# google/zopfli

Measured on AMD Instinct MI355X. Metric: input MB/s at numiterations=15 (gzip, bit-exact vs reference), higher is better.
Workload: dtype u8 (f32/f64 cost DP); 1 GPU; class-T synthetic (text-like, the enwik8 stand-in) 100000000 B per GPU, numiterations=15, blocksplitting=0, gzip, BASELINE configs[1]; total_bytes=100000000, master_blocks=100, gather=none (one rank)

## Files before the change

### zopfli_amd/csrc/device/zmx_hip.hip

```cpp
#include <hip/hip_runtime.h>

#include <algorithm>
#include <atomic>
#include <cmath>
#include <cstdio>
#include <cstdlib>
#include <cstring>
#include <mutex>
#include <string>
#include <unordered_map>
#include <vector>

#include "zmx_kernels.h"
#include "zmx_match2.h"
#ifdef ZMX_EXPERIMENTS
#include "zmx_match3.h"
#include "zmx_match4.h"
#else
#define BK_CH 32768u
#endif
#include "zmx_match5.h"
#include "zmx_dp4.h"
#include "zmx_dp5.h"
#include "zmx_encode.h"
// ... 540 lines not shown
#ifdef ZMX_EXPERIMENTS
  HIPCHK(hipFuncSetAttribute(reinterpret_cast<const void*>(k_bucket), hipFuncAttributeMaxDynamicSharedMemorySize,
                             BK_LDS_BYTES));
#endif
  *out = c;
  return 0;
}

int zmx_ctx_set_priority(zmx_ctx* c, int level) {
  DeviceGuard dev_guard(c->device);
  HIPCHK(dev_guard.err);
  const int k = level > 0 ? 1 : level < 0 ? 2 : 0;
  if (!c->alt_stream[0][0]) { c->alt_stream[0][0] = c->stream; c->alt_stream[0][1] = c->stream2; }
  if (k && !c->alt_stream[k][1]) {
    int least = 0, greatest = 0;
    HIPCHK(hipDeviceGetStreamPriorityRange(&least, &greatest));
    for (int i = 0; i < 2; ++i) {
      if (c->alt_stream[k][i]) continue;
      HIPCHK(hipStreamCreateWithPriority(&c->alt_stream[k][i], hipStreamDefault, k == 1 ? greatest : least));
    }
  }
  HIPCHK(hipStreamSynchronize(c->stream));
  HIPCHK(hipStreamSynchronize(c->stream2));
  c->stream = c->alt_stream[k][0];
  c->stream2 = c->alt_stream[k][1];
  return 0;
}

void zmx_ctx_destroy(zmx_ctx* c) {
  if (!c) return;
  DeviceGuard dev_guard(c->device);
  if (c->h_stage) (void)hipHostFree(c->h_stage);
  for (auto& f : c->pinned_free) (void)hipHostFree(f.first);
  for (auto& f : c->pool_free) (void)hipFree(f.first);
  DevCached(c).fetch_sub(c->pool_free_bytes, std::memory_order_relaxed);
  for (auto& f : c->pool_live) (void)hipFree(c->guard_live.count(f.first) ? static_cast<unsigned char*>(f.first) - kGuardBytes : f.first);
  (void)hipFree(c->d_guard_tab);
  for (int i = 0; i < 4; ++i) if (c->ev[i]) (void)hipEventDestroy(c->ev[i]);
  for (int i = 0; i < 2; ++i) if (c->ev2[i]) (void)hipEventDestroy(c->ev2[i]);
  if (c->alt_stream[0][0]) {
    for (int k = 0; k < 3; ++k) for (int i = 0; i < 2; ++i) if (c->alt_stream[k][i]) (void)hipStreamDestroy(c->alt_stream[k][i]);
  } else {
    if (c->stream2) (void)hipStreamDestroy(c->stream2);
    if (c->stream) (void)hipStreamDestroy(c->stream);
  }
  delete c;
}

int zmx_set_input(zmx_ctx* c, const unsigned char* in, size_t insize) {
  DeviceGuard dev_guard(c->device);
  HIPCHK(dev_guard.err);
  if (insize + kInputPad > c->in_cap) {
    PoolFree(c, c->d_in);
    c->d_in = nullptr;
    c->in_cap = insize + kInputPad;
    HIPCHK(PoolAllocT(c, &c->d_in, c->in_cap, "d_in"));
  }
  if (insize) HIPCHK(hipMemcpyAsync(c->d_in, in, insize, hipMemcpyHostToDevice, c->stream));
  HIPCHK(hipMemsetAsync(c->d_in + insize, 0, kInputPad, c->stream));
  HIPCHK(hipStreamSynchronize(c->stream));
  c->insize = insize;
  c->h_in = in;
  return 0;
}

static void ReleaseTableArrays(zmx_ctx* c, zmx_tables* t, bool keep_stores) {
  auto rel = [&](auto*& p) { PoolFree(c, p); p = nullptr; };
  rel(t->d_blocks);
  rel(t->d_tile_off);
  rel(t->d_same16);
  rel(t->d_links);
  rel(t->d_sorted_alloc);
  rel(t->d_ssame);
  rel(t->d_chunk_base);
  rel(t->d_recs);
  rel(t->d_pool);
  rel(t->d_la);
  rel(t->d_dph);
  rel(t->d_block_edges);
  rel(t->d_badpos);
  rel(t->d_code_base);
  rel(t->d_codes);
  rel(t->d_wtab);
  rel(t->d_badcodes);
  rel(t->d_seg_off);
  rel(t->d_extab);
  rel(t->d_seginfo);
  rel(t->d_counters);
  rel(t->d_prof);
  rel(t->d_tasks);
  rel(t->d_task_off);
  rel(t->d_wg_tasks);
  rel(t->d_task_kind);
  rel(t->d_run_list);
  rel(t->d_wmeta);
  rel(t->d_runin);
  rel(t->d_runout);
  rel(t->d_winroff);
  rel(t->d_winflag);
  rel(t->d_win_off);
  rel(t->d_lvl);
  rel(t->d_entry);
  rel(t->d_exit);
  rel(t->d_mid);
  rel(t->d_chk);
  rel(t->d_over);
  rel(t->d_redo);
  for (int h = 0; h < 2; ++h) { rel(t->d_rank[h]); rel(t->d_bucket[h]); }
  t->d_sorted[0] = t->d_sorted[1] = nullptr;
  PinnedGive(c, &t->h_runin, t->h_runin_cap);
  PinnedGive(c, &t->h_runout, t->h_runout_cap);
  if (!keep_stores) { rel(t->d_store[0]); rel(t->d_store[1]); }
}

void zmx_tables_free(zmx_ctx* c, zmx_tables* t) {
  if (!t) return;
  DeviceGuard dev_guard(c ? c->device : 0);
  if (c && c->stream2) (void)hipStreamSynchronize(c->stream2);
  ReleaseTableArrays(c, t, false);
  delete t;
}

int zmx_tables_trim(zmx_ctx* c, zmx_tables* t) {
  if (!t) return 0;
  DeviceGuard dev_guard(c->device);
  HIPCHK(dev_guard.err);
  HIPCHK(hipStreamSynchronize(c->stream));
  HIPCHK(hipStreamSynchronize(c->stream2));
  ReleaseTableArrays(c, t, true);
  t->trimmed = true;
  return 0;
}

static unsigned EnvU32(const char* name, unsigned dflt, unsigned lo, unsigned hi) {
  const char* e = std::getenv(name);
  if (!e) return dflt;
  const long v = std::atol(e);
  return v < static_cast<long>(lo) ? lo : v > static_cast<long>(hi) ? hi : static_cast<unsigned>(v);
}
static unsigned SegL(u64 total_positions) {
  static const bool set = std::getenv("ZOPFLI_AMD_SEG_L") != nullptr;
  static const unsigned v = EnvU32("ZOPFLI_AMD_SEG_L", 4096, 0, 1u << 24) & ~63u;
  if (set) return v;
  return total_positions <= (128u << 10) ? 256u : total_positions <= (16u << 20) ? 512u : total_positions <= (48u << 20) ? 1024u : 2048u;
}
static unsigned SegHead(size_t nb) {
  static const unsigned v = EnvU32("ZOPFLI_AMD_SEG_HEAD", 0, 0, 1u << 24) & ~63u;
  return v ? v : (nb >= 48 ? 8192u : 0u);
}
static unsigned SegWarm() { static const unsigned v = (EnvU32("ZOPFLI_AMD_SEG_WARM", 512, 64, 1u << 20) + 63u) & ~63u; return v; }

static int BuildTables(zmx_ctx* c, const zmx_block* blocks, size_t nb, zmx_tables* t, zmx_tables* parent = nullptr, bool with_dp = true) {
  const int mk = MatchKernel();
  t->matches_only = !with_dp;
  t->nb = nb;
  t->blocks.resize(nb);
  t->bsize.resize(nb);
  t->store_begin[0].assign(nb, 0);
  t->store_begin[1].assign(nb, 0);
  std::vector<u32> tile_off(nb + 1, 0);
  u64 pos_off = 0, reg_off = 0, la_off = 0, max_l = 0;
  for (size_t b = 0; b < nb; ++b) {
    if (blocks[b].inend < blocks[b].instart || blocks[b].inend > c->insize) {
      return FailMsg("zmx_tables_build: block outside the resident input");
    }
    BlockDesc& d = t->blocks[b];
    d.instart = blocks[b].instart;
    d.inend = blocks[b].inend;
    d.ws = d.instart > ZMX_WINDOW ? d.instart - ZMX_WINDOW : 0;
    d.pos_off = pos_off;
    d.reg_off = reg_off;
    d.la_off = la_off;
    const u64 B = d.inend - d.instart, L = d.inend - d.ws;
    if (B > 0x7fff0000ull) return FailMsg("zmx_tables_build: block too large (positions are 32-bit)");
    t->bsize[b] = static_cast<u32>(B);
    pos_off += B;
    reg_off += (L + 7) & ~7ull;
    la_off += (B + 1 + 7) & ~7ull;
    max_l = std::max(max_l, L);
    tile_off[b + 1] = tile_off[b] + static_cast<u32>((B + MT - 1) / MT);
  }
  t->total_b = pos_off;
  t->total_l = reg_off;
  t->tile_off = tile_off;
  if (nb == 0) return 0;

  std::vector<u64> src_pos;
  std::vector<u64> link_lo;
  std::vector<u32> tile_list;
  bool reuse = parent != nullptr && parent->nb > 0 && c->h_in != nullptr && parent->d_recs != nullptr &&
               parent->total_b + pos_off < (3ull << 30);
  if (reuse) {
    src_pos.resize(nb);
    link_lo.resize(nb);
    size_t pb = 0;
    for (size_t b = 0; b < nb && reuse; ++b) {
      const BlockDesc& d = t->blocks[b];
      while (pb < parent->nb && parent->blocks[pb].inend < d.inend) ++pb;
      if (pb == parent->nb || d.instart < parent->blocks[pb].instart || d.inend > parent->blocks[pb].inend) {
        reuse = false;
        break;
      }
      const BlockDesc& pd = parent->blocks[pb];
      src_pos[b] = pd.pos_off + (d.instart - pd.instart);
      const u64 B = d.inend - d.instart;
      link_lo[b] = d.inend - d.ws;
      if (B == 0 || d.inend == pd.inend) continue;
      u64 t0 = B > ZMX_MAX_MATCH ? d.inend - ZMX_MAX_MATCH : d.instart;
      const unsigned char lastb = c->h_in[d.inend - 1];
      u64 r = d.inend - 1;
      while (r > d.instart && d.inend - r < 65600 && c->h_in[r - 1] == lastb) --r;
      if (r < t0) t0 = r;
      const u32 tile_first = static_cast<u32>((t0 - d.instart) / MT);
      for (u32 tile = tile_first; tile < tile_off[b + 1] - tile_off[b]; ++tile) {
        tile_list.push_back(tile_off[b] + tile);
      }
      const u64 first_index = d.instart + static_cast<u64>(tile_first) * MT - d.ws;
      link_lo[b] = first_index > ZMX_WINDOW ? first_index - ZMX_WINDOW : 0;
    }
  }

  HIPCHK(PoolAlloc(c, &t->d_blocks, nb));
  HIPCHK(PoolAlloc(c, &t->d_tile_off, nb + 1));
  HIPCHK(PoolAlloc(c, &t->d_same16, reg_off));
#ifdef ZMX_EXPERIMENTS
  t->buckets = mk == 3 || mk == 4;
#else
  t->buckets = false;
#endif
  t->chunk_base.assign(nb + 1, 0);
  for (size_t b = 0; b < nb; ++b) {
    const u64 L = t->blocks[b].inend - t->blocks[b].ws;
    t->chunk_base[b + 1] = t->chunk_base[b] + static_cast<u32>((L + BK_CH - 1) / BK_CH);
  }
#ifdef ZMX_EXPERIMENTS
  if (t->buckets) {
    HIPCHK(PoolAlloc(c, &t->d_sorted_alloc, 2 * reg_off + 2 * M4_PAD));
    t->d_sorted[0] = t->d_sorted_alloc + M4_PAD;
    t->d_sorted[1] = t->d_sorted[0] + reg_off + M4_PAD;
    for (int h = 0; h < 2; ++h) {
      HIPCHK(PoolAlloc(c, &t->d_rank[h], reg_off));
      HIPCHK(PoolAlloc(c, &t->d_bucket[h], static_cast<size_t>(t->chunk_base[nb]) * 32768u));
    }
    HIPCHK(PoolAlloc(c, &t->d_ssame, reg_off));
    HIPCHK(PoolAlloc(c, &t->d_chunk_base, nb + 1));
    HIPCHK(hipMemcpyAsync(t->d_chunk_base, t->chunk_base.data(), (nb + 1) * sizeof(u32), hipMemcpyHostToDevice, c->stream));
  } else
#endif
  {
    HIPCHK(PoolAlloc(c, &t->d_links, reg_off));
  }
  HIPCHK(PoolAlloc(c, &t->d_recs, pos_off * 8));
  HIPCHK(PoolAlloc(c, &t->d_la, la_off));
  HIPCHK(PoolAlloc(c, &t->d_store[0], pos_off));
  HIPCHK(PoolAlloc(c, &t->d_store[1], pos_off));
  {
    const size_t in_cost = 0, in_min = in_cost + nb * ZMX_HIST * sizeof(double), in_info = in_min + nb * sizeof(double),
                 in_slot = in_info + 3 * nb * sizeof(float);
    t->runin_bytes = in_slot + nb * sizeof(int);
    const size_t out_hist = 0, out_nsym = out_hist + nb * ZMX_HIST * sizeof(u32), out_stats = out_nsym + nb * sizeof(u32),
                 out_flags = out_stats + 8 * sizeof(u32);
    t->runout_bytes = out_flags + 4 * sizeof(u32);
    HIPCHK(PoolAlloc(c, &t->d_runin, t->runin_bytes));
    HIPCHK(PoolAlloc(c, &t->d_runout, t->runout_bytes));
    HIPCHK(PinnedTake(c, &t->h_runin, t->runin_bytes, &t->h_runin_cap));
    HIPCHK(PinnedTake(c, &t->h_runout, t->runout_bytes, &t->h_runout_cap));
    t->d_cost = reinterpret_cast<double*>(t->d_runin + in_cost);
    t->d_mincost = reinterpret_cast<double*>(t->d_runin + in_min);
    t->d_runinfo = reinterpret_cast<float*>(t->d_runin + in_info);
    t->d_slot = reinterpret_cast<int*>(t->d_runin + in_slot);
    t->d_hist = reinterpret_cast<u32*>(t->d_runout + out_hist);
    t->d_nsym = reinterpret_cast<u32*>(t->d_runout + out_nsym);
    t->d_segstats = reinterpret_cast<u32*>(t->d_runout + out_stats);
    t->d_flags = reinterpret_cast<u32*>(t->d_runout + out_flags);
    HIPCHK(hipMemsetAsync(t->d_segstats, 0, 12 * sizeof(u32), c->stream));
  }
  HIPCHK(PoolAlloc(c, &t->d_dph, pos_off));
  HIPCHK(PoolAlloc(c, &t->d_block_edges, nb));
  t->badpos_words = pos_off / 32 + 4;
  HIPCHK(PoolAlloc(c, &t->d_badpos, t->badpos_words));
  HIPCHK(PoolAlloc(c, &t->d_code_base, nb));
  HIPCHK(PoolAlloc(c, &t->d_wtab, nb * ZMX_WTAB));
  HIPCHK(PoolAlloc(c, &t->d_badcodes, nb * 40));
  HIPCHK(PoolAlloc(c, &t->d_counters, 48));
  HIPCHK(hipMemcpyAsync(t->d_blocks, t->blocks.data(), nb * sizeof(BlockDesc), hipMemcpyHostToDevice, c->stream));
  HIPCHK(hipMemcpyAsync(t->d_tile_off, tile_off.data(), (nb + 1) * sizeof(u32), hipMemcpyHostToDevice, c->stream));
  HIPCHK(hipMemsetAsync(t->d_flags, 0, 4 * sizeof(u32), c->stream));

  HIPCHK(hipEventRecord(c->ev[0], c->stream));
  PoolScope hash_tmp(c);
  u16* d_lev = nullptr;
  u16* d_tot2 = nullptr;
  u16* d_rank2 = nullptr;
  uint4* d_xrec = nullptr;
  u32* d_tot12 = nullptr;
  unsigned long long* d_energy = nullptr;
  u32* d_cmax = nullptr;
  bool skip_any = false, skip_all = false;
  double skip_positions = 0;
  unsigned long long* d_m5stats = nullptr;
  bool join_stream2 = false;
  auto launch_hash = [&](const u64* d_link_lo) -> int {
    if (max_l == 0) return 0;
    const dim3 g1(static_cast<unsigned>((max_l + 256 * SAME_CH - 1) / (256 * SAME_CH)), static_cast<unsigned>(nb));
    hipLaunchKernelGGL(k_same, g1, dim3(256), 0, c->stream, c->d_in, t->d_blocks, t->d_same16, d_link_lo);
    KCHK(c, "k_same");
    HIPCHK(hipGetLastError());
    const dim3 g2(static_cast<unsigned>((max_l + CH_EMIT - 1) / CH_EMIT), static_cast<unsigned>(nb), 2);
#ifdef ZMX_EXPERIMENTS
    if (t->buckets) {
      BucketParams kp;
      kp.in = c->d_in;
      kp.blocks = t->d_blocks;
      kp.same16 = t->d_same16;
      kp.chunk_base = t->d_chunk_base;
      kp.link_lo = d_link_lo;
      for (int h = 0; h < 2; ++h) { kp.sorted[h] = t->d_sorted[h]; kp.rank[h] = t->d_rank[h]; kp.bucket[h] = t->d_bucket[h]; }
      kp.ssame = t->d_ssame;
      hipLaunchKernelGGL(k_bucket, g2, dim3(BK_THREADS), BK_LDS_BYTES, c->stream, kp);
      KCHK(c, "k_bucket");
    } else
#endif
    {
      hipLaunchKernelGGL(k_chain, g2, dim3(64), CH_LDS_BYTES, c->stream, c->d_in, t->d_blocks, t->d_same16, t->d_links, d_link_lo);
      KCHK(c, "k_chain");
      if ((mk == 5 || mk == 0) && d_link_lo == nullptr) {
        skip_any = mk == 5;
        if (mk == 5) for (size_t b = 0; b < nb; ++b) skip_positions += static_cast<double>(t->blocks[b].inend - t->blocks[b].instart);
        const unsigned hits_chunks = static_cast<unsigned>((max_l + RK_CH - 1) / RK_CH);
        {
          static const bool rank_all = [] { const char* e = std::getenv("ZOPFLI_AMD_RANK_ALL"); return e && std::atoi(e) != 0; }();
          if (!d_energy) HIPCHK(hash_tmp.AllocT(&d_energy, nb, "d_energy"));
          if (!d_cmax && !rank_all) HIPCHK(hash_tmp.AllocT(&d_cmax, nb * static_cast<size_t>(hits_chunks) + 1, "d_cmax"));
          HIPCHK(hipMemsetAsync(d_energy, 0, nb * sizeof(unsigned long long), c->stream));
          if (d_cmax) HIPCHK(hipMemsetAsync(d_cmax, 0, (nb * static_cast<size_t>(hits_chunks) + 1) * sizeof(u32), c->stream));
          HitsParams hp;
          hp.in = c->d_in;
          hp.blocks = t->d_blocks;
          hp.same16 = t->d_same16;
          hp.energy = d_energy;
          hp.cmax = d_cmax;
          const dim3 g5(hits_chunks, static_cast<unsigned>(nb));
          hipLaunchKernelGGL(k_hits, g5, dim3(RK_THREADS), 0, c->stream, hp);
          KCHK(c, "k_hits");
        }
        if (mk == 0) {
          std::vector<unsigned long long> energy(nb);
          HIPCHK(hipMemcpyAsync(energy.data(), d_energy, nb * sizeof(unsigned long long), hipMemcpyDeviceToHost, c->stream));
          HIPCHK(hipStreamSynchronize(c->stream));
          size_t on = 0;
          for (size_t b = 0; b < nb; ++b) {
            if (energy[b] > MatchAutoHits() * (t->blocks[b].inend - t->blocks[b].ws)) {
              ++on;
              skip_positions += static_cast<double>(t->blocks[b].inend - t->blocks[b].instart);
            }
          }
          skip_any = on != 0;
          skip_all = on == nb;
        }
        if (skip_any) {
          if (!d_lev) HIPCHK(hash_tmp.AllocT(&d_lev, static_cast<size_t>(LV_N) * reg_off, "d_lev"));
          if (!d_tot2) HIPCHK(hash_tmp.AllocT(&d_tot2, 2 * reg_off, "d_tot"));
          if (!d_rank2) HIPCHK(hash_tmp.AllocT(&d_rank2, 2 * reg_off, "d_rank"));
          if (!d_tot12) HIPCHK(hash_tmp.AllocT(&d_tot12, reg_off, "d_tot12"));
          if (!d_xrec) HIPCHK(hash_tmp.AllocT(&d_xrec, 2 * reg_off, "d_xrec"));
          LevelParams lp;
          lp.in = c->d_in;
          lp.blocks = t->d_blocks;
          lp.lev = d_lev;
          lp.total_l = reg_off;
          lp.energy = mk == 0 ? d_energy : nullptr;
          lp.thr = MatchAutoHits();
          const dim3 g4(static_cast<unsigned>((max_l + LV_CH - 1) / LV_CH), static_cast<unsigned>(nb), LV_N);
          hipLaunchKernelGGL(k_levels, g4, dim3(64), 0, c->stream, lp);
          KCHK(c, "k_levels");
          RankParams rp;
          rp.in = c->d_in;
          rp.blocks = t->d_blocks;
          rp.links = t->d_links;
          rp.same16 = t->d_same16;
          rp.lev = d_lev;
          rp.total_l = reg_off;
          rp.tot = d_tot2;
          rp.rank = d_rank2;
          rp.xrec = d_xrec;
          rp.tot12 = d_tot12;
          rp.energy = lp.energy;
          rp.thr = lp.thr;
          rp.cmax = d_cmax;
          rp.cmax_stride = hits_chunks;
          const dim3 g3(static_cast<unsigned>((max_l + RK_CH - 1) / RK_CH), static_cast<unsigned>(nb));
          hipLaunchKernelGGL(k_rank2, g3, dim3(RK_THREADS), 0, c->stream, rp);
          KCHK(c, "k_rank2");
        }
      }
    }
    return 0;
  };
  {
    u64* d_link_lo = nullptr;
    if (reuse) {
      HIPCHK(hash_tmp.AllocT(&d_link_lo, nb, "d_link_lo"));
      HIPCHK(hipMemcpyAsync(d_link_lo, link_lo.data(), nb * sizeof(u64), hipMemcpyHostToDevice, c->stream));
    }
    if (launch_hash(d_link_lo) != 0) return -1;
    t->links_partial = reuse;
  }

  if (mk != 3 && !c->d_scratch) HIPCHK(PoolAllocT(c, &c->d_scratch, static_cast<size_t>(kMatchGrid) * M2_THREADS * SCRATCH_CPS, "d_scratch"));
  HIPCHK(hipEventRecord(c->ev[1], c->stream));
  double match_positions = 0;
  double m5_lane_iters = 0, m5_iters = 0;
  auto launch_match = [&](u32* pool, u32 pool_cap, u32 total_tiles, const u32* d_tiles, bool prof) -> int {
    if (total_tiles == 0) return 0;
#ifdef ZMX_EXPERIMENTS
    if (t->buckets) {
      Match3Params mp;
      mp.in = c->d_in;
      mp.blocks = t->d_blocks;
      mp.tile_off = t->d_tile_off;
      mp.nb = static_cast<u32>(nb);
      mp.total_tiles = total_tiles;
      mp.same16 = t->d_same16;
      mp.chunk_base = t->d_chunk_base;
      for (int h = 0; h < 2; ++h) { mp.sorted[h] = t->d_sorted[h]; mp.rank[h] = t->d_rank[h]; mp.bucket[h] = t->d_bucket[h]; }
      mp.ssame = t->d_ssame;
      mp.recs = t->d_recs;
      mp.pool = pool;
      mp.pool_cap = pool_cap;
      mp.counters = t->d_counters;
      mp.tile_list = d_tiles;
      mp.scratch = c->d_scratch;
      if (mk == 3) {
        if (prof) hipLaunchKernelGGL((k_match3<true>), dim3(kMatchGrid3), dim3(M3_THREADS), 0, c->stream, mp);
        else hipLaunchKernelGGL((k_match3<false>), dim3(kMatchGrid3), dim3(M3_THREADS), 0, c->stream, mp);
        KCHK(c, "k_match3");
      } else {
        if (prof) hipLaunchKernelGGL((k_match4<true>), dim3(kMatchGrid3), dim3(M4_THREADS), 0, c->stream, mp);
        else hipLaunchKernelGGL((k_match4<false>), dim3(kMatchGrid3), dim3(M4_THREADS), 0, c->stream, mp);
        KCHK(c, "k_match4");
      }
      return 0;
    }
#endif
    MatchParams mp;
    mp.in = c->d_in;
    mp.blocks = t->d_blocks;
    mp.tile_off = t->d_tile_off;
    mp.nb = static_cast<u32>(nb);
    mp.total_tiles = total_tiles;
    mp.links = t->d_links;
    mp.recs = t->d_recs;
    mp.pool = pool;
    mp.pool_cap = pool_cap;
    mp.counters = t->d_counters;
    mp.scratch = c->d_scratch;
    mp.tile_list = d_tiles;
    mp.skip_energy = nullptr;
    mp.skip_thr = 0;
    if ((mk == 5 || mk == 0) && d_tiles == nullptr && skip_any) {
      if (!c->d_scratch5) HIPCHK(PoolAllocT(c, &c->d_scratch5, static_cast<size_t>(kMatchGrid5) * M5_THREADS * SCRATCH_CPS, "d_scratch5"));
      Match5Params q;
      q.m = mp;
      q.m.scratch = c->d_scratch5;
      q.xrec = d_xrec;
      q.tot12 = d_tot12;
      q.energy = mk == 0 ? d_energy : nullptr;
      q.thr = MatchAutoHits();
      const size_t m5_waves = static_cast<size_t>(kMatchGrid5) * (M5_THREADS / 64);
      if (!d_m5stats) HIPCHK(hash_tmp.AllocT(&d_m5stats, 2 * m5_waves, "d_m5stats"));
      HIPCHK(hipMemsetAsync(d_m5stats, 0, 2 * m5_waves * sizeof(unsigned long long), c->stream));
      q.wave_stats = d_m5stats;
      {
        static const int forced = [] { const char* e = std::getenv("ZOPFLI_AMD_M5_UNIT"); return e ? std::atoi(e) : -1; }();
        const u64 waves = static_cast<u64>(kMatchGrid5) * (M5_THREADS / 64);
        q.sub_shift = forced >= 0 ? static_cast<u32>(forced > 2 ? 2 : forced) : (mp.total_tiles >= 4 * waves ? 1u : 2u);
      }
      if (mk == 5 || skip_all) {
        hipLaunchKernelGGL(k_match5, dim3(kMatchGrid5), dim3(M5_THREADS), 0, c->stream, q);
        KCHK(c, "k_match5");
        return 0;
      }
      HIPCHK(hipEventRecord(c->ev2[0], c->stream));
      HIPCHK(hipStreamWaitEvent(c->stream2, c->ev2[0], 0));
      hipLaunchKernelGGL(k_match5, dim3(kMatchGrid5), dim3(M5_THREADS), 0, c->stream2, q);
      HIPCHK(hipGetLastError());
      c->stream2_outstanding = true;
      HIPCHK(hipEventRecord(c->ev2[1], c->stream2));
      join_stream2 = true;
      mp.skip_energy = d_energy;
      mp.skip_thr = MatchAutoHits();
    }
    const bool filt = MatchFilter();
    if (prof && filt) hipLaunchKernelGGL((k_match2<true, true>), dim3(kMatchGrid), dim3(M2_THREADS), 0, c->stream, mp);
    else if (prof) hipLaunchKernelGGL((k_match2<true, false>), dim3(kMatchGrid), dim3(M2_THREADS), 0, c->stream, mp);
    else if (filt) hipLaunchKernelGGL((k_match2<false, true>), dim3(kMatchGrid), dim3(M2_THREADS), 0, c->stream, mp);
    else hipLaunchKernelGGL((k_match2<false, false>), dim3(kMatchGrid), dim3(M2_THREADS), 0, c->stream, mp);
    if (join_stream2) {
      join_stream2 = false;
      HIPCHK(hipStreamWaitEvent(c->stream, c->ev2[1], 0));
      c->stream2_outstanding = false;
    }
    KCHK(c, "k_match2");
    return 0;
  };

  if (reuse) {
    u64* d_src_pos = nullptr;
    u32* d_tile_list = nullptr;
    PoolScope tmp(c);
    HIPCHK(tmp.AllocT(&d_src_pos, nb, "d_src_pos"));
    HIPCHK(tmp.AllocT(&d_tile_list, tile_list.size(), "d_tile_list"));
    HIPCHK(hipMemcpyAsync(d_src_pos, src_pos.data(), nb * sizeof(u64), hipMemcpyHostToDevice, c->stream));
    if (!tile_list.empty()) {
      HIPCHK(hipMemcpyAsync(d_tile_list, tile_list.data(), tile_list.size() * sizeof(u32), hipMemcpyHostToDevice, c->stream));
    }
    CopyRecsParams cp;
    cp.blocks = t->d_blocks;
    cp.src_pos = d_src_pos;
    cp.src = reinterpret_cast<const uint4*>(parent->d_recs);
    cp.dst = reinterpret_cast<uint4*>(t->d_recs);
    u64 max_b = 0;
    for (size_t b = 0; b < nb; ++b) max_b = std::max<u64>(max_b, t->bsize[b]);
    const unsigned gx = static_cast<unsigned>(std::min<u64>(std::max<u64>((max_b * 2 + 256 * 16 - 1) / (256 * 16), 1), 4096));
    hipLaunchKernelGGL(k_copy_recs, dim3(gx, static_cast<unsigned>(nb)), dim3(256), 0, c->stream, cp);
    KCHK(c, "k_copy_recs");
    HIPCHK(hipGetLastError());
    HIPCHK(hipMemsetAsync(t->d_counters, 0, 48 * sizeof(u32), c->stream));
    HIPCHK(hipMemcpyAsync(t->d_counters, parent->d_counters, sizeof(u32), hipMemcpyDeviceToDevice, c->stream));
    if (launch_match(parent->d_pool, parent->pool_cap, static_cast<u32>(tile_list.size()), d_tile_list, false) != 0) return -1;
    u32 counters[2] = {0, 0};
    HIPCHK(hipMemcpyAsync(counters, t->d_counters, sizeof(counters), hipMemcpyDeviceToHost, c->stream));
    HIPCHK(hipStreamSynchronize(c->stream));
    if ((counters[1] & 1u) == 0) {
      t->d_pool = parent->d_pool;
      t->pool_cap = parent->pool_cap;
      parent->d_pool = nullptr;
      parent->pool_cap = 0;
    } else {
      reuse = false;
      if (launch_hash(nullptr) != 0) return -1;
      t->links_partial = false;
    }
  }

  static const u64 pool_entries = [] { const char* e = std::getenv("ZOPFLI_AMD_POOL_ENTRIES"); return e ? static_cast<u64>(std::atoll(e)) : 0ull; }();
  u64 per_pos = 4;
  for (bool first_try = true; !reuse; first_try = false) {
    u64 cap = std::max<u64>(pos_off * per_pos, 1u << 16);
    if (first_try && pool_entries) cap = pool_entries;
    if (cap > 0xfffffff0ull) cap = 0xfffffff0ull;
    PoolFree(c, t->d_pool);
    t->d_pool = nullptr;
    HIPCHK(PoolAlloc(c, &t->d_pool, cap));
    t->pool_cap = static_cast<u32>(cap);
    HIPCHK(hipMemsetAsync(t->d_counters, 0, 48 * sizeof(u32), c->stream));
    static const bool match_prof = std::getenv("ZOPFLI_AMD_PROF") != nullptr;
    if (launch_match(t->d_pool, t->pool_cap, tile_off[nb], nullptr, match_prof) != 0) return -1;
    u32 counters[2] = {0, 0};
    HIPCHK(hipMemcpyAsync(counters, t->d_counters, sizeof(counters), hipMemcpyDeviceToHost, c->stream));
    HIPCHK(hipStreamSynchronize(c->stream));
    match_positions += static_cast<double>(pos_off);
    if (d_m5stats) {
      const size_t m5_waves = static_cast<size_t>(kMatchGrid5) * (M5_THREADS / 64);
      std::vector<unsigned long long> ws(2 * m5_waves);
      HIPCHK(hipMemcpy(ws.data(), d_m5stats, ws.size() * sizeof(unsigned long long), hipMemcpyDeviceToHost));
      m5_lane_iters = m5_iters = 0;
      for (size_t w = 0; w < m5_waves; ++w) { m5_lane_iters += static_cast<double>(ws[2 * w]); m5_iters += static_cast<double>(ws[2 * w + 1]); }
    }
    if (counters[1] & 2u) {
      u32 dbg[8] = {0};
      HIPCHK(hipMemcpy(dbg, t->d_counters + 32, sizeof(dbg), hipMemcpyDeviceToHost));
      char buf[320];
      std::snprintf(buf, sizeof(buf), "zmx_tables_build: k_match5's wave loop did not end (state %08x xd %u curd %u bestlen %u limit %u nlink %u eqd %u "
                    "li %u idx %u same %u cur %u bestdist %u)", dbg[0], dbg[1], dbg[2], dbg[3] & 0xffffu, dbg[3] >> 16, dbg[4] & 0xffffu, dbg[4] >> 16,
                    dbg[5], dbg[6] & 0xffffu, dbg[6] >> 16, dbg[7] & 0xffffu, dbg[7] >> 16);
      return FailFault(buf);
    }
    if ((counters[1] & 1u) == 0) break;
    if (per_pos >= 256) return FailMsg("zmx_tables_build: change-point pool overflow");
    per_pos *= 8;
  }
  {
    HIPCHK(hipEventRecord(c->ev[2], c->stream));
    HIPCHK(hipEventSynchronize(c->ev[2]));
    float ms_hash = 0, ms_match = 0;
    HIPCHK(hipEventElapsedTime(&ms_hash, c->ev[0], c->ev[1]));
    HIPCHK(hipEventElapsedTime(&ms_match, c->ev[1], c->ev[2]));
    g_match_stats[0] += ms_match * 1e-3;
    g_match_stats[1] += ms_hash * 1e-3;
    g_match_stats[2] += 1;
    g_match_stats[3] += reuse ? static_cast<double>(tile_list.size()) * MT : match_positions;
    if (skip_any && !reuse) {
      g_match5_stats[0] += m5_lane_iters;
      g_match5_stats[1] += m5_iters;
      g_match5_stats[2] += skip_positions;
    }
    if (std::getenv("ZOPFLI_AMD_PROF") && !reuse) {
      unsigned long long hc[2] = {0, 0};
      HIPCHK(hipMemcpy(hc, t->d_counters + 4, sizeof(hc), hipMemcpyDeviceToHost));
      const double pos = static_cast<double>(pos_off);
      std::fprintf(stderr, "%s: %.2f ms for %.0f positions: %.1f chain hits per "
                   "position, %.1f of 64 lanes with a hit per wave-loop iteration; %.1f SIMD cycles per hit (2.4 GHz, 1024 SIMDs)\n", mk == 5 || mk == 0 ? "k_match5 / k_match2 (hits = entries touched)" : mk == 4 ? "k_match4" : mk == 3 ? "k_match3" : "k_match2", ms_match, pos,
                   static_cast<double>(hc[0]) / pos, static_cast<double>(hc[0]) / static_cast<double>(hc[1] ? hc[1] : 1),
                   ms_match * 1e-3 * 2.4e9 * 1024 / static_cast<double>(hc[0] ? hc[0] : 1));
      if (mk == 3) {
        unsigned long long h3[3] = {0, 0, 0};
        HIPCHK(hipMemcpy(h3, t->d_counters + 16, sizeof(h3), hipMemcpyDeviceToHost));
// ... 1307 lines not shown
```

### zopfli_amd/csrc/device/zmx_kernels.h

```cpp
#pragma once
#include <hip/hip_runtime.h>
#include <stdint.h>

typedef unsigned char u8;
typedef unsigned short u16;
typedef unsigned int u32;
typedef unsigned long long u64;

struct BlockDesc {
  u64 instart, inend, ws;
  u64 pos_off;
  u64 reg_off;
  u64 la_off;
};

#define ZMX_WINDOW 32768u
#define ZMX_MAX_MATCH 258u
#define ZMX_MAX_CHAIN_HITS 8192
#define ZMX_NONE16 0xffffu

__device__ __forceinline__ int dev_dist_symbol(u32 d) {
  if (d < 5) return (int)d - 1;
  const int l = 31 - __clz((int)(d - 1));
  return 2 * l + (int)(((d - 1) >> (l - 1)) & 1);
}
__device__ __forceinline__ int dev_dist_extra_bits(u32 d) {
  return d < 5 ? 0 : (31 - __clz((int)(d - 1))) - 1;
}
__device__ __forceinline__ int dev_length_symbol(u32 l) {
  if (l < 11) return 254 + (int)l;
  if (l == 258) return 285;
  const int e = 31 - __clz((int)(l - 3)) - 2;
  return 261 + 4 * e + (int)(((l - 3) >> e) & 3);
}
__device__ __forceinline__ int dev_length_extra_bits(u32 l) {
  if (l < 11 || l == 258) return 0;
  return 31 - __clz((int)(l - 3)) - 2;
}

#define ZMX_WAVE_SCAN(NAME, OP, IDENT)                                                   \
  __device__ __forceinline__ u32 NAME(u32 v) {                                           \
    u32 t;                                                                               \
    t = (u32)__builtin_amdgcn_update_dpp((int)(IDENT), (int)v, 0x111, 0xf, 0xf, false); v = OP(v, t); \
    t = (u32)__builtin_amdgcn_update_dpp((int)(IDENT), (int)v, 0x112, 0xf, 0xf, false); v = OP(v, t); \
    t = (u32)__builtin_amdgcn_update_dpp((int)(IDENT), (int)v, 0x114, 0xf, 0xf, false); v = OP(v, t); \
    t = (u32)__builtin_amdgcn_update_dpp((int)(IDENT), (int)v, 0x118, 0xf, 0xf, false); v = OP(v, t); \
    t = (u32)__builtin_amdgcn_update_dpp((int)(IDENT), (int)v, 0x142, 0xa, 0xf, false); v = OP(v, t); \
    t = (u32)__builtin_amdgcn_update_dpp((int)(IDENT), (int)v, 0x143, 0xc, 0xf, false); v = OP(v, t); \
    return v;                                                                            \
  }
__device__ __forceinline__ u32 zmx_addu(u32 a, u32 b) { return a + b; }
__device__ __forceinline__ u32 zmx_maxu(u32 a, u32 b) { return a > b ? a : b; }
ZMX_WAVE_SCAN(wave_scan_add, zmx_addu, 0u)
ZMX_WAVE_SCAN(wave_scan_max, zmx_maxu, 0u)

__device__ __forceinline__ u32 rdlane_u32(u32 v, u32 l) { return (u32)__builtin_amdgcn_readlane((int)v, (int)l); }
__device__ __forceinline__ float rdlane_f32(float v, u32 l) {
  return __int_as_float(__builtin_amdgcn_readlane(__float_as_int(v), (int)l));
}
__device__ __forceinline__ void wave_lds_sync() {
  __builtin_amdgcn_fence(__ATOMIC_ACQ_REL, "wavefront");
  __builtin_amdgcn_wave_barrier();
}

#define SAME_CH 64

__global__ __launch_bounds__(256) void k_same(const u8* __restrict__ in, const BlockDesc* __restrict__ blocks,
                                              u16* __restrict__ same16, const u64* __restrict__ link_lo) {
  const BlockDesc bd = blocks[blockIdx.y];
  const u64 L = bd.inend - bd.ws;
  const u64 c0 = ((u64)blockIdx.x * blockDim.x + threadIdx.x) * SAME_CH;
  if (c0 >= L) return;
  const u64 c1 = (c0 + SAME_CH < L) ? c0 + SAME_CH : L;
  if (link_lo) {
    const u64 lo = link_lo[blockIdx.y];
    if (lo >= L) return;
    const u64 chunk0 = lo / 32768u * 32768u;
    if (c1 + 32768u <= chunk0) return;
  }
  const u8* base = in + bd.ws;
  u32 next = 0;
  if (c1 < L) {
    const u8 c = base[c1];
    u64 q = c1 + 1;
    u32 r = 0;
    bool stop = false;
    while (q < L && r < 65535u && (((u64)(base + q)) & 7)) {
      if (base[q] != c) { stop = true; break; }
      ++q; ++r;
    }
    if (!stop) {
      const u64 pat = 0x0101010101010101ull * c;
      while (q + 8 <= L && r < 65535u) {
        const u64 x = *reinterpret_cast<const u64*>(base + q) ^ pat;
        if (x) { r += (u32)(__ffsll((long long)x) - 1) >> 3; stop = true; break; }
        q += 8; r += 8;
      }
      if (!stop) {
        while (q < L && r < 65535u && base[q] == c) { ++q; ++r; }
      }
    }
    next = r < 65535u ? r : 65535u;
  }
  u16* out = same16 + bd.reg_off;
  for (u64 k = c1; k-- > c0;) {
    u32 s = 0;
    if (k + 1 < L && base[k + 1] == base[k]) s = next < 65535u ? next + 1 : 65535u;
    out[k] = (u16)s;
    next = s;
  }
}

#define CH_EMIT 32768u
#define CH_TILE 1024u
#define CH_LDS_BYTES (65536 + CH_TILE * 4)

__global__ __launch_bounds__(64) void k_chain(const u8* __restrict__ in, const BlockDesc* __restrict__ blocks,
                                              const u16* __restrict__ same16, ushort4* __restrict__ links,
                                              const u64* __restrict__ link_lo) {
  extern __shared__ __align__(16) u8 dyn_lds[];
  u16* head = reinterpret_cast<u16*>(dyn_lds);
  u16* keys = head + 32768;
  u16* sames = keys + CH_TILE;

  const BlockDesc bd = blocks[blockIdx.y];
  const u32 chain = blockIdx.z;
  const u64 L = bd.inend - bd.ws;
  const u64 e0 = (u64)blockIdx.x * CH_EMIT;
  if (e0 >= L) return;
  const u64 e1 = (e0 + CH_EMIT < L) ? e0 + CH_EMIT : L;
  if (link_lo && e1 <= link_lo[blockIdx.y]) return;
  const u64 w0 = e0 >= ZMX_WINDOW ? e0 - ZMX_WINDOW : 0;
  const u32 lane = threadIdx.x;
  const u64 lt_mask = (1ull << lane) - 1;
  const u64 gt_mask = ~((2ull << lane) - 1);

  for (u32 i = lane; i < 16384; i += 64) reinterpret_cast<u32*>(head)[i] = 0xffffffffu;
  __syncthreads();

  const u8* base = in + bd.ws;
  const u16* same = same16 + bd.reg_off;
  ushort4* lk = links + bd.reg_off;

  for (u64 t0 = w0; t0 < e1; t0 += CH_TILE) {
    const u32 tn = (u32)((e1 - t0 < CH_TILE) ? e1 - t0 : CH_TILE);
    {
      const u32 i0 = 16u * lane;
      u32 by[18];
      u32 sm[16];
#pragma unroll
      for (u32 q = 0; q < 18; ++q) {
        const u64 k = t0 + i0 + q;
        by[q] = (i0 < tn && k < L) ? (u32)base[k] : 0u;
      }
#pragma unroll
      for (u32 q = 0; q < 16; ++q) sm[q] = (i0 + q < tn) ? (u32)same[t0 + i0 + q] : 0u;
#pragma unroll
      for (u32 q = 0; q < 16; ++q) {
        if (i0 + q < tn) {
          u32 v = ((by[q] << 10) ^ (by[q + 1] << 5) ^ by[q + 2]) & 32767u;
          if (chain) v ^= (sm[q] - 3u) & 255u;
          keys[i0 + q] = (u16)v;
          sames[i0 + q] = (u16)sm[q];
        }
      }
    }
    __syncthreads();
    const u32 cur0 = (u32)(t0 - w0);
    for (u32 i0 = 0; i0 < tn; i0 += 64) {
      const u32 i = i0 + lane;
      const bool act = i < tn;
      const u32 key = act ? (u32)keys[i] : 0u;
      if (t0 + i0 + 64 <= e0) {
        const u32 r = cur0 + i;
        bool todo = act;
        while (__any(todo)) {
          if (todo) head[key] = (u16)r;
          wave_lds_sync();
          const u32 w = act ? (u32)head[key] : 0xffffu;
          wave_lds_sync();
          todo = act && w < r;
        }
        continue;
      }
      const u32 old = act ? (u32)head[key] : (u32)ZMX_NONE16;
      u64 grp = __ballot(act);
#pragma unroll
      for (int bit = 0; bit < 15; ++bit) {
        const bool mine = (key >> bit) & 1;
        const u64 bm = __ballot(mine);
        grp &= mine ? bm : ~bm;
      }
      const u64 lower = grp & lt_mask;
      const u32 r = cur0 + i;
      u32 d;
      if (lower) d = lane - (63u - (u32)__clzll((long long)lower));
      else d = old == ZMX_NONE16 ? 0u : r - old;
      if (d > 32767u) d = 0;
      wave_lds_sync();
      if (act && (grp & gt_mask) == 0) head[key] = (u16)r;
      wave_lds_sync();
      const u64 k = t0 + i;
      if (act && k >= e0) {
        if (chain == 0) {
          lk[k].x = (u16)d;
          lk[k].z = sames[i];
        } else {
          lk[k].y = (u16)d;
        }
      }
    }
    __syncthreads();
  }
}

#define MT 2048u
#define MWIN_BYTES (32768u + MT + 288u)
#define SCRATCH_CPS 256u
#define M_XCD_GROUP 16u
#define MATCH_BATCH 8u

struct MatchParams {
  const u8* in;
  const BlockDesc* blocks;
  const u32* tile_off;
  u32 nb;
  u32 total_tiles;
  const ushort4* links;
  u32* recs;
  u32* pool;
  u32 pool_cap;
  u32* counters;
  u32* scratch;
  const u32* tile_list;
  const unsigned long long* skip_energy;
  u64 skip_thr;
};

__device__ __forceinline__ u32 lds_byte(const u32* w, u32 a) { return reinterpret_cast<const u8*>(w)[a]; }
__device__ __forceinline__ u32 lds_u32_unaligned(const u32* w, u32 a) {
  const u32 lo = w[a >> 2], hi = w[(a >> 2) + 1];
  return __builtin_amdgcn_alignbyte(hi, lo, a & 3);
}

struct CopyRecsParams {
  const BlockDesc* blocks;
  const u64* src_pos;
  const uint4* src;
  uint4* dst;
};

__global__ __launch_bounds__(256) void k_copy_recs(CopyRecsParams P) {
  const BlockDesc bd = P.blocks[blockIdx.y];
  const u64 n = (u64)(bd.inend - bd.instart) * 2;
  const uint4* src = P.src + P.src_pos[blockIdx.y] * 2;
  uint4* dst = P.dst + bd.pos_off * 2;
  for (u64 i = (u64)blockIdx.x * 256 + threadIdx.x; i < n; i += (u64)gridDim.x * 256) dst[i] = src[i];
}

__device__ __forceinline__ u32 rec_dist_for(const u32* __restrict__ rec, const u32* __restrict__ pool, u32 len) {
  const u32 d1 = rec[1];
  const u32 ncpf = d1 >> 24;
  if (ncpf != 0xffu) {
    const u8* b = reinterpret_cast<const u8*>(rec) + 8;
    for (u32 e = 0; e < ncpf; ++e) {
      if ((u32)b[3 * e] + 3u >= len) return (u32)b[3 * e + 1] | ((u32)b[3 * e + 2] << 8);
    }
    return 0;
  }
  const u32 off = rec[2], n = rec[3] & 0xffffu;
  for (u32 e = 0; e < n; ++e) {
    const u32 x = pool[off + e];
    if ((x & 0xffffu) >= len) return x >> 16;
  }
  return 0;
}

__device__ __forceinline__ void hist_add_symbol(u32* hist, u32 litlen, u32 dist) {
  if (dist == 0) {
    atomicAdd(&hist[litlen], 1u);
  } else {
    atomicAdd(&hist[dev_length_symbol(litlen)], 1u);
    atomicAdd(&hist[288 + dev_dist_symbol(dist)], 1u);
  }
}

__device__ __forceinline__ uint2 greedy_window(const u32* rbase, u32 wb, u32 lane, u32 B) {
  const u32 q = wb + lane < B ? wb + lane : (B ? B - 1 : 0);
  return *reinterpret_cast<const uint2*>(rbase + (u64)q * 8);
}

#define TR_CHUNK 2048u

struct RowScanParams {
  const BlockDesc* blocks;
  const u32* recs;
  uint2* dph;
  u64* block_edges;
  u32 codeless;
};
#define DPH_CODELESS (1u << 26)
__device__ __forceinline__ u32 dph_layout_len(u32 y) { return (y & DPH_CODELESS) ? 0u : (y & 0xffffu); }

__global__ __launch_bounds__(1024) void k_rowscan(RowScanParams P) {
  __shared__ u32 s_wsum[16];
  const BlockDesc bd = P.blocks[blockIdx.x];
  const u32 B = (u32)(bd.inend - bd.instart);
  const u32 tid = threadIdx.x, lane = tid & 63, wid = tid >> 6;
  const u32* rbase = P.recs + bd.pos_off * 8;
  uint2* out = P.dph + bd.pos_off;
  u64 carry = 0;
  for (u32 t0 = 0; t0 < B; t0 += 1024) {
    const u32 jj = t0 + tid;
    const bool act = jj < B;
    u32 kend = 0, sflag = 0;
    if (act) {
      const uint2 h = *reinterpret_cast<const uint2*>(rbase + (u64)jj * 8);
      const u32 leng = h.x & 0xffffu, same_i = h.y & 0xffffu;
      if (leng >= 3 && (h.x >> 16) == 1u && (h.y >> 24) == 1u) sflag |= 2u;
      sflag |= ((h.y >> 16) & 255u) << 2;
      kend = leng < B - jj ? leng : B - jj;
      if (kend < 3) kend = 1;
      if (same_i > 2 * ZMX_MAX_MATCH && jj > ZMX_MAX_MATCH + 1 && jj + 2 * ZMX_MAX_MATCH + 1 < B) {
        const u32 same_back = rbase[(u64)(jj - ZMX_MAX_MATCH) * 8 + 1] & 0xffffu;
        sflag |= same_back > ZMX_MAX_MATCH ? 1u : 0u;
      }
    }
    const bool nocodes = P.codeless != 0 && (sflag & 2u) != 0 && kend >= 64u;
    const u32 klay = nocodes ? 0u : kend;
    const u32 incl = wave_scan_add(klay);
    if (lane == 63) s_wsum[wid] = incl;
    __syncthreads();
    u32 woff = 0, tot = 0;
#pragma unroll
    for (u32 w = 0; w < 16; ++w) {
      const u32 v = s_wsum[w];
      if (w < wid) woff += v;
      tot += v;
    }
    if (act) out[jj] = make_uint2((u32)carry + woff + incl - klay, kend | (sflag << 16) | (nocodes ? DPH_CODELESS : 0u));
    carry += tot;
    __syncthreads();
  }
  if (tid == 0) P.block_edges[blockIdx.x] = carry;
}

#define EG_CAP 2048u
#define ZMX_NUM_W 1127u
#define ZMX_WTAB 1152u

__device__ __forceinline__ u32 weight_code(u32 k, u32 dist) {
  return (257u + 30u * (u32)(dev_length_symbol(k) - 257) + (u32)dev_dist_symbol(dist)) * 8u;
}

struct CodeParams {
  const BlockDesc* blocks;
  const u32* tile_off;
  u32 nb_total;
  const u32* recs;
  const u32* pool;
  const uint2* dph;
  u16* codes;
  const u64* code_base;
};

__global__ __launch_bounds__(256) void k_codes(CodeParams P) {
  __shared__ u8 s_mark[4][EG_CAP];
  __shared__ u32 s_hoff[4][64];
  __shared__ u32 s_hthr[4][64][2];
  __shared__ u16 s_hdist[4][64][8];
  __shared__ u32 s_hpool[4][64][2];

  const u32 tid = threadIdx.x, lane = tid & 63, wid = tid >> 6;
  const u32 tile = blockIdx.x;
  u32 lo = 0, hi = P.nb_total;
  while (hi - lo > 1) {
    const u32 mid = (lo + hi) >> 1;
    if (P.tile_off[mid] <= tile) lo = mid; else hi = mid;
  }
  const u32 b = lo;
  const BlockDesc bd = P.blocks[b];
  const u32 B = (u32)(bd.inend - bd.instart);
  const u32 tp0 = (tile - P.tile_off[b]) * MT;
  const u32* rbase = P.recs + bd.pos_off * 8;
  const uint2* dbase = P.dph + bd.pos_off;
  u16* codes = P.codes + P.code_base[b];
  u8* mark = s_mark[wid];

  for (u32 g = wid; g < MT / 64; g += 4) {
    const u32 base = tp0 + g * 64;
    if (base >= B) break;
    const u32 navail = (B - base < 64u) ? B - base : 64u;
    const u32 jj = base + lane;
    const bool act = lane < navail;
    uint4 ra = make_uint4(0, 0, 0, 0), rb = make_uint4(0, 0, 0, 0);
    uint2 dh = make_uint2(0, 0);
    if (act) {
      ra = *reinterpret_cast<const uint4*>(rbase + (u64)jj * 8);
      rb = *reinterpret_cast<const uint4*>(rbase + (u64)jj * 8 + 4);
      dh = dbase[jj];
    }
    const u32 lit = (ra.y >> 16) & 255u;
    const u32 ncpf = ra.y >> 24;
    const u32 kend = dh.y & 0xffffu;
    const u32 klay = dph_layout_len(dh.y);
    const u32 off = dh.x;
    const u32 offend = off + (act ? klay : 0u);
    const u32 off0 = rdlane_u32(off, 0);

    wave_lds_sync();
    {
      const bool ovf = ncpf == 0xffu;
// ... 196 lines not shown
```

Before: 792.2 MB/s.

## Parallelize k_same run-length computation with wave scan and vectorized stores

Reworks the same-byte run-length kernel so each thread handles 8 bytes instead of 64, with per-block stretches resolved by a wave-level max scan plus a cross-wave LDS carry. A single wave probes past the stretch end cooperatively using ballot over 64 lanes of 8-byte loads. Outputs are written as 16-byte vector stores. This targets the long serial per-thread loops and uncoalesced writes of the old kernel, at the cost of extra synchronization and scan logic.

```diff
diff --git a/zopfli_amd/csrc/device/zmx_hip.hip b/zopfli_amd/csrc/device/zmx_hip.hip
--- a/zopfli_amd/csrc/device/zmx_hip.hip
+++ b/zopfli_amd/csrc/device/zmx_hip.hip
@@ -866,8 +866,8 @@
   bool join_stream2 = false;
   auto launch_hash = [&](const u64* d_link_lo) -> int {
     if (max_l == 0) return 0;
-    const dim3 g1(static_cast<unsigned>((max_l + 256 * SAME_CH - 1) / (256 * SAME_CH)), static_cast<unsigned>(nb));
-    hipLaunchKernelGGL(k_same, g1, dim3(256), 0, c->stream, c->d_in, t->d_blocks, t->d_same16, d_link_lo);
+    const dim3 g1(static_cast<unsigned>((max_l + SAME_STRETCH - 1) / SAME_STRETCH), static_cast<unsigned>(nb));
+    hipLaunchKernelGGL(k_same, g1, dim3(SAME_TPB), 0, c->stream, c->d_in, t->d_blocks, t->d_same16, d_link_lo);
     KCHK(c, "k_same");
     HIPCHK(hipGetLastError());
     const dim3 g2(static_cast<unsigned>((max_l + CH_EMIT - 1) / CH_EMIT), static_cast<unsigned>(nb), 2);
diff --git a/zopfli_amd/csrc/device/zmx_kernels.h b/zopfli_amd/csrc/device/zmx_kernels.h
--- a/zopfli_amd/csrc/device/zmx_kernels.h
+++ b/zopfli_amd/csrc/device/zmx_kernels.h
@@ -63,51 +63,102 @@
   __builtin_amdgcn_wave_barrier();
 }
 
-#define SAME_CH 64
-
-__global__ __launch_bounds__(256) void k_same(const u8* __restrict__ in, const BlockDesc* __restrict__ blocks,
-                                              u16* __restrict__ same16, const u64* __restrict__ link_lo) {
+#define SAME_PER 8u
+#define SAME_TPB 256u
+#define SAME_STRETCH (SAME_PER * SAME_TPB)
+
+__global__ __launch_bounds__(SAME_TPB) void k_same(const u8* __restrict__ in, const BlockDesc* __restrict__ blocks,
+                                                   u16* __restrict__ same16, const u64* __restrict__ link_lo) {
+  __shared__ u32 s_probe;
+  __shared__ u32 s_wave[SAME_TPB / 64];
   const BlockDesc bd = blocks[blockIdx.y];
   const u64 L = bd.inend - bd.ws;
-  const u64 c0 = ((u64)blockIdx.x * blockDim.x + threadIdx.x) * SAME_CH;
-  if (c0 >= L) return;
-  const u64 c1 = (c0 + SAME_CH < L) ? c0 + SAME_CH : L;
+  const u64 s0 = (u64)blockIdx.x * SAME_STRETCH;
+  if (s0 >= L) return;
+  const u64 s1 = (s0 + SAME_STRETCH < L) ? s0 + SAME_STRETCH : L;
   if (link_lo) {
     const u64 lo = link_lo[blockIdx.y];
     if (lo >= L) return;
     const u64 chunk0 = lo / 32768u * 32768u;
-    if (c1 + 32768u <= chunk0) return;
+    if (s1 + 32768u <= chunk0) return;
   }
   const u8* base = in + bd.ws;
-  u32 next = 0;
-  if (c1 < L) {
-    const u8 c = base[c1];
-    u64 q = c1 + 1;
-    u32 r = 0;
-    bool stop = false;
-    while (q < L && r < 65535u && (((u64)(base + q)) & 7)) {
-      if (base[q] != c) { stop = true; break; }
-      ++q; ++r;
-    }
-    if (!stop) {
-      const u64 pat = 0x0101010101010101ull * c;
-      while (q + 8 <= L && r < 65535u) {
-        const u64 x = *reinterpret_cast<const u64*>(base + q) ^ pat;
-        if (x) { r += (u32)(__ffsll((long long)x) - 1) >> 3; stop = true; break; }
-        q += 8; r += 8;
-      }
-      if (!stop) {
-        while (q < L && r < 65535u && base[q] == c) { ++q; ++r; }
-      }
-    }
-    next = r < 65535u ? r : 65535u;
-  }
-  u16* out = same16 + bd.reg_off;
-  for (u64 k = c1; k-- > c0;) {
-    u32 s = 0;
-    if (k + 1 < L && base[k + 1] == base[k]) s = next < 65535u ? next + 1 : 65535u;
-    out[k] = (u16)s;
-    next = s;
+  const u32 tid = threadIdx.x, lane = tid & 63u, wid = tid >> 6;
+
+  if (wid == 0) {
+    u32 e = (u32)(s1 - s0);
+    if (s1 < L) {
+      const u64 qmax = (s1 + 65536u < L) ? s1 + 65536u : L;
+      const u64 pat = 0x0101010101010101ull * base[s1];
+      u64 found = qmax;
+      const u64 q0 = s1 + 1;
+      for (u64 a = q0 - (((u64)(base + q0)) & 7u); a < qmax; a += 512) {
+        const u64 w = a + 8u * lane;
+        u64 hit = ~0ull;
+        if (w < qmax) {
+          u64 x = *reinterpret_cast<const u64*>(base + w) ^ pat;
+          if (w < q0) x &= ~0ull << (8u * (u32)(q0 - w));
+          if (w + 8 > qmax) x &= (1ull << (8u * (u32)(qmax - w))) - 1;
+          if (x) hit = w + ((u32)(__ffsll((long long)x) - 1) >> 3);
+        }
+        const u64 m = __ballot(hit != ~0ull);
+        if (m) {
+          const u32 l = (u32)__builtin_ctzll(m);
+          found = ((u64)rdlane_u32((u32)(hit >> 32), l) << 32) | rdlane_u32((u32)hit, l);
+          break;
+        }
+      }
+      e = (u32)(found - s0);
+    }
+    if (lane == 0) s_probe = e;
+  }
+
+  const u32 ci = wid * 64u + (63u - lane);
+  const u64 k0 = s0 + (u64)ci * SAME_PER;
+  u32 chg = 0;
+  if (k0 < L) {
+    u32 prev = base[k0];
+#pragma unroll
+    for (u32 j = 1; j <= SAME_PER; ++j) {
+      const u64 q = k0 + j;
+      u32 c = 0;
+      if (q < L) c = base[q];
+      if (q >= L || c != prev) chg |= 1u << j;
+      prev = c;
+    }
+  }
+  const u32 f = chg ? (u32)(k0 - s0) + (u32)__builtin_ctz(chg) : 0xffffffffu;
+  const u32 incl = wave_scan_max(~f);
+  u32 excl = __shfl_up(incl, 1, 64);
+  if (lane == 0) excl = 0u;
+  if (lane == 63) s_wave[wid] = incl;
+  __syncthreads();
+  u32 carry = ~s_probe;
+#pragma unroll
+  for (u32 w = 0; w < SAME_TPB / 64; ++w) {
+    if (w > wid) carry = carry > s_wave[w] ? carry : s_wave[w];
+  }
+  if (k0 >= L) return;
+  u32 e = ~(excl > carry ? excl : carry);
+  u32 sv[SAME_PER];
+#pragma unroll
+  for (int j = (int)SAME_PER - 1; j >= 0; --j) {
+    const u32 k = (u32)(k0 - s0) + (u32)j;
+    if ((chg >> (j + 1)) & 1u) e = k + 1u;
+    const u32 r = e - k - 1u;
+    sv[j] = r < 65535u ? r : 65535u;
+  }
+  u16* out = same16 + bd.reg_off + k0;
+  if (k0 + SAME_PER <= L) {
+    uint4 v;
+    v.x = sv[0] | (sv[1] << 16); v.y = sv[2] | (sv[3] << 16);
+    v.z = sv[4] | (sv[5] << 16); v.w = sv[6] | (sv[7] << 16);
+    *reinterpret_cast<uint4*>(out) = v;
+  } else {
+#pragma unroll
+    for (u32 j = 0; j < SAME_PER; ++j) {
+      if (k0 + j < L) out[j] = (u16)sv[j];
+    }
   }
 }
 
```

After: 800.0 MB/s, median of 5. No clear change (+1.0%).
